# paulvoliva/XNODE-WAN-PDE-solver

Measured on AMD Instinct MI355X. Metric: WAN training-steps/sec (optimiser sub-steps, d=20 cube, N_r=4096 paths per GPU), higher is better.
Workload: dtype f64

## Files before the change

xnode_wan_pde_solver_amd/csrc/xw_ode_mfma4.h:

```cpp
#if XW_ODE_SECTION == 1
static_assert(XW_ODE_K <= 15, "row K of the 16-row K-tile is the ones row that collects the bias gradients");
static_assert(Dim<XW_ODE_H, XW_ODE_K>::HT <= 2 && Dim<XW_ODE_H, XW_ODE_K>::CT <= 3, "H <= 32");
template <int H, int K> struct FieldW {
  double Wy[Dim<H, K>::KB][Dim<H, K>::HB];
  double Wh[Dim<H, K>::KB][Dim<H, K>::KB];
  double Wo[Dim<H, K>::HB][Dim<H, K>::KB];
  d4 wt, bh;
  d4 bo[Dim<H, K>::HT];
};
template <int H, int K> struct FieldWT {
  double WyT[Dim<H, K>::HB][Dim<H, K>::KB];
  double WhT[Dim<H, K>::KB][Dim<H, K>::KB];
  double WoT[Dim<H, K>::KB][Dim<H, K>::HB];
};
template <int H, int K>
__device__ __forceinline__ void load_field(const double* __restrict__ th, const UOff& o, int d, FieldW<H, K>& w) {
  typedef Dim<H, K> D;
  const double* Wy = th + o.Win + d + 1;
#pragma unroll
  for (int rb = 0; rb < D::KB; ++rb) {
#pragma unroll
    for (int kb = 0; kb < D::HB; ++kb) w.Wy[rb][kb] = xw_fragA4(Wy, o.ldin, K, H, 4 * rb, 4 * kb);
#pragma unroll
    for (int kb = 0; kb < D::KB; ++kb) w.Wh[rb][kb] = xw_fragA4(th + o.Wh, K, K, K, 4 * rb, 4 * kb);
// ... 232 lines not shown
  const long col = (long)tile * 16 + 4 * k + b;
  const double* __restrict__ src_y = s.Yl + (long)row * N + (col < N - 1 ? col : N - 1);
  const double* __restrict__ src_a = s.A + (long)(AL::YI + (s.i > 0 ? s.i - 1 : 0) * H + 4 * cb) * 16 + lane;
  const xw_gptr src = row < H ? (xw_gptr)(first ? src_y : src_a) : (xw_gptr)&xw_duo_const[0][0];
  return __builtin_nontemporal_load(src);
}
__device__ __forceinline__ double duo_readA(const double* tile, int rb) {
  const int l = xw_lane();
  return tile[(4 * rb + (l & 3)) * XW_TSTRIDE + ((l >> 2) & 3) * 4 + (l >> 4)];
}
__device__ __forceinline__ double duo_fold(double x) {
  x += __shfl_xor(x, 4);
  x += __shfl_xor(x, 8);
  return x;
}
template <int H, int K, int M, int METHOD>
__device__ __forceinline__ void duo_outer(const BwdJobs& jobs, const double* __restrict__ tf, const double* __restrict__ th,
                                          int L, int d, const double* qbuf, int vb) {
  typedef Dim<H, K> D;
  typedef RK<METHOD> T;
  typedef DuoPlan<H, K, M> P;
  typedef Duo4<H, K, M> Q;
  typedef DuoSrc<H, K, M, METHOD> Src;
  constexpr int NH = M > 1 ? M - 1 : 1;
  xw_setprio(jobs.prio);
  const int job = find_job(jobs, vb);
  const double* __restrict__ Y = jobs.Y[job];
  const double* __restrict__ act = jobs.act[job];
  const int N = jobs.N[job];
  const int tile = vb - jobs.tile0[job];
  const int lane = xw_lane();
  const UOff o = u_offsets(d, H, K);
  double gWh[Q::KB][Q::KB1], gWo[Q::HB][Q::KB1], gWy[Q::KB][Q::HB1];
#pragma unroll
  for (int rb = 0; rb < Q::KB; ++rb) {
#pragma unroll
    for (int cb = 0; cb < Q::KB1; ++cb) gWh[rb][cb] = 0.0;
#pragma unroll
    for (int cb = 0; cb < Q::HB1; ++cb) gWy[rb][cb] = 0.0;
  }
#pragma unroll
  for (int rb = 0; rb < Q::HB; ++rb)
#pragma unroll
    for (int cb = 0; cb < Q::KB1; ++cb) gWo[rb][cb] = 0.0;
  double Ra[Q::KB1], Rr[NH][Q::KB1], Ry[Q::HB1];
  const int E = (L - 1) * T::S;
  double ti_cur = 0.0;
  if (E > 0) {
    const Src s0(Y, act, tf, 0, L, N, tile);
    ti_cur = s0.ti;
#pragma unroll
    for (int cb = 0; cb < Q::KB1; ++cb) Ra[cb] = duo_load_act<H, K, M, METHOD>(s0, M - 1, cb);
#pragma unroll
    for (int jj = M - 2; jj >= 0; --jj)
#pragma unroll
      for (int cb = 0; cb < Q::KB1; ++cb) Rr[jj][cb] = duo_load_act<H, K, M, METHOD>(s0, jj, cb);
#pragma unroll
    for (int cb = 0; cb < Q::HB1; ++cb) Ry[cb] = duo_load_y<H, K, M, METHOD>(s0, cb, N, tile);
  }
  const bool trow = (lane & 3) == (H & 3);
  for (int e = 0; e < E; ++e) {
    asm volatile("s_barrier" ::: "memory");
    const double* q = qbuf + (e & 1) * P::BUF;
    const Src sn(Y, act, tf, e + 1 < E ? e + 1 : e, L, N, tile);
    double Ao[Q::HB], Az[M][Q::KB];
#pragma unroll
    for (int rb = 0; rb < Q::HB; ++rb) Ao[rb] = duo_readA(q + P::off(rb >> 2), rb & 3);
#pragma unroll
    for (int tq = 0; tq < M; ++tq)
#pragma unroll
      for (int rb = 0; rb < Q::KB; ++rb) Az[tq][rb] = duo_readA(q + P::off(D::HT + tq), rb);
    __builtin_amdgcn_sched_barrier(0);
#pragma unroll
    for (int cb = 0; cb < Q::KB1; ++cb)
#pragma unroll
      for (int rb = 0; rb < Q::HB; ++rb) gWo[rb][cb] = XW_MFMA4(Ao[rb], Ra[cb], gWo[rb][cb]);
    __builtin_amdgcn_sched_barrier(0);
#pragma unroll
    for (int cb = 0; cb < Q::KB1; ++cb) Ra[cb] = duo_load_act<H, K, M, METHOD>(sn, M - 1, cb);
    __builtin_amdgcn_sched_barrier(0);
#pragma unroll
    for (int jj = M - 2; jj >= 0; --jj) {
#pragma unroll
      for (int cb = 0; cb < Q::KB1; ++cb)
#pragma unroll
        for (int rb = 0; rb < Q::KB; ++rb) gWh[rb][cb] = XW_MFMA4(Az[M - 2 - jj][rb], Rr[jj][cb], gWh[rb][cb]);
      __builtin_amdgcn_sched_barrier(0);
#pragma unroll
      for (int cb = 0; cb < Q::KB1; ++cb) Rr[jj][cb] = duo_load_act<H, K, M, METHOD>(sn, jj, cb);
      __builtin_amdgcn_sched_barrier(0);
    }
#pragma unroll
    for (int cb = 0; cb < Q::HB1; ++cb) {
      const double b = (cb == (H >> 2) && trow) ? ti_cur : Ry[cb];
#pragma unroll
      for (int rb = 0; rb < Q::KB; ++rb) gWy[rb][cb] = XW_MFMA4(Az[M - 1][rb], b, gWy[rb][cb]);
    }
    __builtin_amdgcn_sched_barrier(0);
#pragma unroll
    for (int cb = 0; cb < Q::HB1; ++cb) Ry[cb] = duo_load_y<H, K, M, METHOD>(sn, cb, N, tile);
    __builtin_amdgcn_sched_barrier(0);
    ti_cur = sn.ti;
  }
  double* slab = jobs.gslab[job] + (long)tile * o.total;
  const int i = lane >> 4, j = lane & 3;
  const bool owner = ((lane >> 2) & 3) == 0;
#pragma unroll
  for (int rb = 0; rb < Q::KB; ++rb)
#pragma unroll
    for (int cb = 0; cb < Q::KB1; ++cb) {
      const double x = duo_fold(gWh[rb][cb]);
      const int row = 4 * rb + i, col = 4 * cb + j;
      if (owner && row < K) {
        if (col < K) slab[o.Wh + row * K + col] = x;
        else if (col == K) slab[o.Whb + row] = x;
      }
    }
#pragma unroll
  for (int rb = 0; rb < Q::HB; ++rb)
#pragma unroll
    for (int cb = 0; cb < Q::KB1; ++cb) {
      const double x = duo_fold(gWo[rb][cb]);
      const int row = 4 * rb + i, col = 4 * cb + j;
      if (owner && row < H) {
        if (col < K) slab[o.Wo + row * K + col] = x;
        else if (col == K) slab[o.Wob + row] = x;
      }
    }
#pragma unroll
  for (int rb = 0; rb < Q::KB; ++rb)
#pragma unroll
    for (int cb = 0; cb < Q::HB1; ++cb) {
      const double x = duo_fold(gWy[rb][cb]);
      const int row = 4 * rb + i, col = 4 * cb + j;
      if (owner && row < K) {
        if (col < H) slab[o.Win + row * o.ldin + d + 1 + col] = x;
        else if (col == H) slab[o.Win + row * o.ldin + d] = x;
      }
    }
}
#elif XW_ODE_SECTION == 3
#include "xw_ode_n4.h"

template <int H, int K, int M>
bool launch_fwd_narrow(int sel, const FwdJobs& jobs, const double* t, const double* theta, int L, int d, dim3 grid, hipStream_t s, int& rc) {
  if (!jobs.narrow) return false;
  rc = XW_E_ARG;
// ... 6 lines not shown
    case 5: hipLaunchKernelGGL((n4::k_ode_fwd_n4<H, K, M, 1, 2>), grid, dim3(256), 0, s, jobs, t, theta, L, d); break;
    case 6: hipLaunchKernelGGL((n4::k_ode_fwd_n4<H, K, M, 2, 0>), grid, dim3(256), 0, s, jobs, t, theta, L, d); break;
    default: return true;
  }
  rc = xw_launch_status();
  return true;
}
template <int H, int K, int M, bool PARAMS>
int launch_bwd(int method, const BwdJobs& jobs, const double* t, const double* theta, int L, int d, bool adj, bool narrow,
               hipStream_t s) {
  const dim3 grid(jobs.tile0[jobs.n]), block(64);
  if (narrow) {
    if (adj || method > 1) return XW_E_ARG;
    for (int i = 0; i < jobs.n; ++i)
      if (jobs.act[i] == nullptr) return XW_E_ARG;
    if (method == 0) hipLaunchKernelGGL((n4::k_ode_bwd_n4<H, K, M, 0, PARAMS>), grid, dim3(256), 0, s, jobs, t, theta, L, d);
    else hipLaunchKernelGGL((n4::k_ode_bwd_n4<H, K, M, 1, PARAMS>), grid, dim3(256), 0, s, jobs, t, theta, L, d);
    return xw_launch_status();
  }
  bool act = true;
  for (int i = 0; i < jobs.n; ++i) act = act && jobs.act[i] != nullptr;
  if (adj || !act || method > 1)
    return XW_ODE_FN(xw_ode_bwd_recomp_w)(&jobs, t, theta, method, L, d, M, PARAMS ? 1 : 0, adj ? 1 : 0, (void*)s);
  static const int spread_on = [] { const char* e = getenv("XW_DUO_SPREAD"); return e ? atoi(e) : 1; }();
  static const int ncu = [] { int dev = 0, n = 0; if (hipGetDevice(&dev) != hipSuccess || hipDeviceGetAttribute(&n, hipDeviceAttributeMultiprocessorCount, dev) != hipSuccess) n = 0; return n; }();
  const int tiles = jobs.tile0[jobs.n];
  BwdJobs jd = jobs;
  jd.spread = (spread_on && ncu > 0 && tiles > ncu && tiles <= 2 * ncu) ? ncu : 0;
  const int rounds = jd.spread ? (tiles + ncu - 1) / ncu : 0;
  const dim3 duo_grid(jd.spread ? (2 * (rounds - 1)) * ncu + (tiles - (rounds - 1) * ncu) : tiles);
// ... 16 lines not shown
```

xnode_wan_pde_solver_amd/csrc/xw_ode_n4.h:

```cpp

namespace n4 {

template <int C> __device__ __forceinline__ int rot_i(int x) {
  if constexpr (C == 0) return x;
  else return __builtin_amdgcn_update_dpp(0, x, 0x120 + 4 * C, 0xf, 0xf, true);
}
template <int C> __device__ __forceinline__ double rot(double x) {
  if constexpr (C == 0) return x;
  else return __hiloint2double(rot_i<C>(__double2hiint(x)), rot_i<C>(__double2loint(x)));
}
struct R4 { double v[4]; };
__device__ __forceinline__ R4 rots(double x) { return R4{{x, rot<1>(x), rot<2>(x), rot<3>(x)}}; }

struct Geo {
  int lo, b, hi;
  int sb[4];
  int q;
};
__device__ __forceinline__ Geo geo() {
  Geo g;
  const int l = xw_lane();
  g.lo = l & 3; g.b = (l >> 2) & 3; g.hi = l >> 4;
  g.sb[0] = g.b; g.sb[1] = rot_i<1>(g.b); g.sb[2] = rot_i<2>(g.b); g.sb[3] = rot_i<3>(g.b);
  g.q = (int)(threadIdx.x >> 6);
// ... 103 lines not shown
  if (PARAMS) {
    R.aT = xw_ld_nt(S + (M - 1) * K * 16 + f.tK);
#pragma unroll
    for (int j = 0; j < M - 1; ++j) R.rT[j] = xw_ld_nt(S + j * K * 16 + f.tK);
    if (i == 0) {
#pragma unroll
      for (int y = 0; y < D::NY; ++y) R.yT[y] = xw_ld_g(Y + (long)l * H * N + yT[y]);
    } else {
#pragma unroll
      for (int y = 0; y < D::NY; ++y) R.yT[y] = xw_ld_nt(A + (long)(AL::YI + (i - 1) * H) * 16 + f.tY[y]);
    }
  }
  __builtin_amdgcn_sched_barrier(0);
}

template <int H, int K, int M, bool PARAMS>
__device__ __forceinline__ void vjp4(const WT4<H, K>& w, double eye, int blk, double t, const Stage4<H, K, M, PARAMS>& s,
                                     const double (&ob)[Dn<H, K>::NY], double (&yb)[Dn<H, K>::NY], double& xpb, Acc4<H, K>& G) {
  typedef Dn<H, K> D;
  __builtin_amdgcn_sched_barrier(0);
  const unsigned bits = s.word << blk;
  double ab = 0.0;
  {
    const R4 o0 = rots(ob[0]);
#pragma unroll
    for (int c = 0; c < 4; ++c) ab = XW_MFMA4(w.WoT0[c], o0.v[c], ab);
    if (D::NY == 2) {
      if (D::REP) ab = XW_MFMA4(w.WoT1[0], ob[D::NY - 1], ab);
      else {
        const R4 o1 = rots(ob[D::NY - 1]);
#pragma unroll
        for (int c = 0; c < 4; ++c) ab = XW_MFMA4(w.WoT1[c], o1.v[c], ab);
      }
    }
  }
  if (PARAMS) {
// ... 4 lines not shown
    G.bo[0] += ob[0];
    if (D::NY == 2) {
      const double q1 = XW_MFMA4(ob[D::NY - 1], eye, 0.0);
      if (D::REP) G.Wo1[0] = XW_MFMA4(q1, aT.v[0], G.Wo1[0]);
      else {
#pragma unroll
        for (int c = 0; c < 4; ++c) G.Wo1[c] = XW_MFMA4(q1, aT.v[c], G.Wo1[c]);
      }
      G.bo[D::NY - 1] += ob[D::NY - 1];
    }
  }
  double zb = ab * fma(-s.a, s.a, 1.0);
#pragma unroll
  for (int j = M - 2; j >= 0; --j) {
    const R4 zr = rots(zb);
    if (PARAMS) {
      const double qz = XW_MFMA4(zb, eye, 0.0);
      const R4 rT = rots(s.rT[j]);
#pragma unroll
      for (int c = 0; c < 4; ++c) G.Wh[c] = XW_MFMA4(qz, rT.v[c], G.Wh[c]);
      G.bh += zb;
    }
    double tt = 0.0;
#pragma unroll
    for (int c = 0; c < 4; ++c) tt = XW_MFMA4(w.WhT[c], zr.v[c], tt);
    zb = Stage4<H, K, M, PARAMS>::gate(bits, j, tt);
  }
  xpb += zb;
  const R4 zr = rots(zb);
  if (PARAMS) {
    const double qz = XW_MFMA4(zb, eye, 0.0);
    const R4 y0 = rots(s.yT[0]);
#pragma unroll
    for (int c = 0; c < 4; ++c) G.Wy0[c] = XW_MFMA4(qz, y0.v[c], G.Wy0[c]);
    if (D::NY == 2) {
      if (D::REP) G.Wy1[0] = XW_MFMA4(qz, s.yT[D::NY - 1], G.Wy1[0]);
      else {
        const R4 y1 = rots(s.yT[D::NY - 1]);
#pragma unroll
        for (int c = 0; c < 4; ++c) G.Wy1[c] = XW_MFMA4(qz, y1.v[c], G.Wy1[c]);
      }
    }
    G.wt = fma(t, zb, G.wt);
  }
#pragma unroll
  for (int y = 0; y < D::NY; ++y) yb[y] = 0.0;
#pragma unroll
  for (int c = 0; c < 4; ++c) {
    yb[0] = XW_MFMA4(w.WyT0[c], zr.v[c], yb[0]);
    if (D::NY == 2) yb[D::NY - 1] = XW_MFMA4(w.WyT1[c], zr.v[c], yb[D::NY - 1]);
  }
}

template <int H, int K> struct Plan4 {
  typedef Dn<H, K> D;
  static constexpr int NG = 12 + 2 * D::NC1;
  static constexpr int NTILE = 2 * D::NY + 2 + D::NY + 1;
  static constexpr int TILES = 0;
  static constexpr int HAND = TILES + XW_SWEEP_TILES * XW_TTILE;
  static constexpr int SCAL = HAND + NTILE * 256;
  static constexpr int GACC = SCAL + 32;
  static constexpr int TOTAL_P = GACC + 4 * NG * 64;
  static constexpr int TOTAL_X = SCAL + 32;
};

__device__ __forceinline__ void hand_over(double* tile, const Geo& g, double x, bool rep) {
  if (!rep) tile[64 * g.b + 16 * g.hi + 4 * g.q + g.lo] = x;
  else tile[64 * g.b + 16 * g.hi + 4 * g.q + g.lo] = g.b == 0 ? x : 0.0;
}
__device__ __forceinline__ d4 take_over(const double* tile) {
  const int l = xw_lane();
  d4 v;
#pragma unroll
  for (int r = 0; r < 4; ++r) v[r] = tile[64 * r + l];
  return v;
}
__device__ __forceinline__ void storeRowSumsStrided(double* dst, long stride, int rows, int r0, d4 q) {
  const int lane = xw_lane(), g = lane >> 4;
#pragma unroll
  for (int r = 0; r < 4; ++r) {
    const double s = xw_sum_over_n(q[r]);
    const int row = r0 + g + 4 * r;
    if ((lane & 15) == 0 && row < rows) dst[(long)row * stride] = s;
  }
}

template <int H, int K, int M, int METHOD, bool PARAMS>
__device__ __forceinline__ void sweep4(const BwdJobs& jobs, const double* __restrict__ tf, const double* __restrict__ th, int L, int d,
                                       double* lds, int vb) {
  typedef Dn<H, K> D;
  typedef Dim<H, K> DW;
  typedef RK<METHOD> T;
  typedef Plan4<H, K> P;
  static_assert(T::S <= 2, "the activation store is used by euler and midpoint");
  static_assert(D::NY == DW::HT, "registers of the hidden state = row tiles of the 16-path layout");
  xw_setprio(jobs.prio);
  const Geo g = geo();
  const int job = find_job(jobs, vb);
  const double* __restrict__ xT = jobs.xT[job];
  const double* __restrict__ start = jobs.start[job];
  const double* __restrict__ Y = jobs.Y[job];
  const double* __restrict__ act = jobs.act[job];
  const int N = jobs.N[job];
  const int tile = vb - jobs.tile0[job];
  const int base = tile * 16;
  const long ntile = (N + 15) >> 4;
  const int colC = base + 4 * g.q + g.lo, colT = base + 4 * g.q + g.hi;
  const bool valid = colC < N;
  const int nclC = valid ? colC : N - 1, nclT = colT < N ? colT : N - 1;
  const UOff o = u_offsets(d, H, K);
  WT4<H, K> w;
  load_WT4<H, K>(th, o, d, g, w);
  const Off4<H, K> f = offsets<H, K>(g);
  const double eye = g.lo == g.hi ? 1.0 : 0.0;
  int rowC[D::NY], rowT[D::NY];
  long yC[D::NY], yT[D::NY];
  double flw[D::NY];
#pragma unroll
  for (int y = 0; y < D::NY; ++y) {
    const int rc = y == 0 ? 4 * g.b + g.hi : (D::REP ? 16 + g.hi : 16 + 4 * g.b + g.hi);
    const int rt = y == 0 ? 4 * g.b + g.lo : (D::REP ? 16 + g.lo : 16 + 4 * g.b + g.lo);
    rowC[y] = rc;
    rowT[y] = rt;
    yC[y] = (long)(rc < H ? rc : H - 1) * N + nclC;
    yT[y] = (long)(rt < H ? rt : H - 1) * N + nclT;
    flw[y] = rc < H ? xw_ld_g(th + o.FLw + rc) : 0.0;
  }
  (void)rowT;

// ... 21 lines not shown
      if (PARAMS) accFL[y] = fma(ub, yl[y], accFL[y]);
    }
    if (PARAMS) accFLb += ub;
  };
  double kb[T::S][D::NY], psum[D::NY];
  auto begin_step = [&](int l) {
    const double dt = tf[l + 1] - tf[l];
#pragma unroll
    for (int i = 0; i < T::S; ++i)
#pragma unroll
      for (int y = 0; y < D::NY; ++y) {
        kb[i][y] = (dt * T::b(i)) * lam[y];
        if (i == 0) psum[y] = 0.0;
      }
  };
  auto reverse_stage = [&](int l, int i, const Stage4<H, K, M, PARAMS>& s) {
    const double t0 = tf[l], dt = tf[l + 1] - t0;
    double psi[D::NY];
    vjp4<H, K, M, PARAMS>(w, eye, g.b, t0 + T::c(i) * dt, s, kb[i], psi, xpb, G);
#pragma unroll
    for (int y = 0; y < D::NY; ++y) {
      psum[y] += psi[y];
#pragma unroll
      for (int j = 0; j < T::S; ++j)
        if (j < i && T::a(i, j) != 0.0) kb[j][y] = fma(dt * T::a(i, j), psi[y], kb[j][y]);
    }
  };
  auto end_step = [&](const double (&yl)[D::NY], double ub) {
#pragma unroll
    for (int y = 0; y < D::NY; ++y) lam[y] += psum[y];
    readout(yl, ub);
  };

  auto run = [&](auto weak_tag) {
    constexpr bool WEAK = decltype(weak_tag)::value;
    Stage4<H, K, M, PARAMS> sa, sb;
    const CotRaw raw_last = cot_issue<WEAK>(cot, L - 1);
    CotRaw raw = cot_issue<WEAK>(cot, L > 1 ? L - 2 : 0);
    if (L > 1) load_stage4<H, K, M, METHOD, PARAMS>(Y, act, L - 2, T::S - 1, N, ntile, tile, g, f, yT, sa);
    {
      double yl[D::NY];
      load_y(L - 1, yl);
      readout(yl, cot_value<WEAK>(cot, raw_last, L - 1, L));
    }
    for (int l = L - 2; l >= 0; --l) {
      const double ub = cot_value<WEAK>(cot, raw, l, L);
      double yl[D::NY];
      load_y(l, yl);
      if constexpr (T::S == 2) {
        load_stage4<H, K, M, METHOD, PARAMS>(Y, act, l, 0, N, ntile, tile, g, f, yT, sb);
        raw = cot_issue<WEAK>(cot, l > 0 ? l - 1 : 0);
        begin_step(l);
        reverse_stage(l, 1, sa);
        load_stage4<H, K, M, METHOD, PARAMS>(Y, act, l > 0 ? l - 1 : 0, 1, N, ntile, tile, g, f, yT, sa);
        reverse_stage(l, 0, sb);
      } else {
        sb = sa;
        raw = cot_issue<WEAK>(cot, l > 0 ? l - 1 : 0);
        load_stage4<H, K, M, METHOD, PARAMS>(Y, act, l > 0 ? l - 1 : 0, 0, N, ntile, tile, g, f, yT, sa);
        begin_step(l);
        reverse_stage(l, 0, sb);
      }
      end_step(yl, ub);
    }
  };
  if (cot.weak) run(std::true_type{});
  else run(std::false_type{});

  double* hand = lds + P::HAND;
#pragma unroll
  for (int y = 0; y < D::NY; ++y) {
    hand_over(hand + (0 * D::NY + y) * 256, g, lam[y], y == 1 && D::REP);
    if (PARAMS) {
      hand_over(hand + (1 * D::NY + y) * 256, g, accFL[y], y == 1 && D::REP);
      hand_over(hand + (2 * D::NY + 2 + y) * 256, g, G.bo[y], y == 1 && D::REP);
    }
  }
  hand_over(hand + (2 * D::NY) * 256, g, xpb, false);
  if (PARAMS) {
    hand_over(hand + (2 * D::NY + 1) * 256, g, G.bh, false);
    hand_over(hand + (3 * D::NY + 2) * 256, g, G.wt, false);
  }
  if (g.b == 0 && g.hi == 0) {
    lds[P::SCAL + 4 * g.q + g.lo] = ub0;
    lds[P::SCAL + 16 + 4 * g.q + g.lo] = accFLb;
  }
  if (PARAMS) {
    double* mine = lds + P::GACC + g.q * (P::NG * 64) + xw_lane();
    int r = 0;
#pragma unroll
    for (int c = 0; c < 4; ++c) mine[64 * (r++)] = G.Wh[c];
#pragma unroll
    for (int c = 0; c < 4; ++c) mine[64 * (r++)] = G.Wo0[c];
#pragma unroll
    for (int c = 0; c < 4; ++c) mine[64 * (r++)] = G.Wy0[c];
#pragma unroll
    for (int c = 0; c < D::NC1; ++c) mine[64 * (r++)] = G.Wo1[c];
#pragma unroll
    for (int c = 0; c < D::NC1; ++c) mine[64 * (r++)] = G.Wy1[c];
  }
  __syncthreads();
  double* slab = PARAMS ? jobs.gslab[job] + (long)tile * o.total : nullptr;
  if (PARAMS) {
    const double* all = lds + P::GACC + xw_lane();
    const int row = 4 * g.b + g.hi;
#pragma unroll
    for (int r = 0; r < P::NG; ++r) {
      if ((r & 3) != g.q) continue;
      const double x = (all[64 * r] + all[64 * (P::NG + r)]) + (all[64 * (2 * P::NG + r)] + all[64 * (3 * P::NG + r)]);
      const int kind = r < 12 ? r >> 2 : 3 + (r - 12) / (D::NC1 > 0 ? D::NC1 : 1);
      const int c = r < 12 ? r & 3 : (r - 12) % (D::NC1 > 0 ? D::NC1 : 1);
      const int col = 4 * g.sb[c] + g.lo;
      if (kind == 0) {
        if (row < K && col < K) slab[o.Wh + row * K + col] = x;
      } else if (kind == 1) {
        if (row < H && col < K) slab[o.Wo + row * K + col] = x;
      } else if (kind == 2) {
        if (row < K && col < H) slab[o.Win + row * o.ldin + d + 1 + col] = x;
// ... 8 lines not shown
  }
  if (g.q != 0) return;
  {
    const int lane = xw_lane(), n = lane & 15;
    const bool valid16 = base + n < N;
    const int ncl16 = valid16 ? base + n : N - 1;
    d4 lam16[DW::HT], fl16[DW::HT], flw16[DW::HT];
#pragma unroll
    for (int ht = 0; ht < DW::HT; ++ht) {
      lam16[ht] = take_over(hand + (0 * D::NY + ht) * 256);
      fl16[ht] = PARAMS ? take_over(hand + (1 * D::NY + ht) * 256) : xw_zero4();
      flw16[ht] = xw_vecD(th + o.FLw, H, 16 * ht);
    }
    const d4 xpb16 = take_over(hand + (2 * D::NY) * 256);
    const double ub016 = lds[P::SCAL + n], flb16 = lds[P::SCAL + 16 + n];
    if (PARAMS) {
      storeRowSums(slab + o.Whb, K, 0, take_over(hand + (2 * D::NY + 1) * 256));
#pragma unroll
      for (int ht = 0; ht < DW::HT; ++ht) storeRowSums(slab + o.Wob, H, 16 * ht, take_over(hand + (2 * D::NY + 2 + ht) * 256));
      storeRowSumsStrided(slab + o.Win + d, o.ldin, K, 0, take_over(hand + (3 * D::NY + 2) * 256));
    }
    sweep_tail<H, K, PARAMS, false>(th, o, d, N, base, valid16, ncl16, xT, start[ncl16], jobs.x_ones != 0, lam16, xpb16, ub016, fl16,
                                    flb16, flw16, jobs.gx[job], jobs.gs[job], slab, lds + P::TILES, []() {});
  }
}

template <int H, int K, int M, int METHOD, bool PARAMS>
__global__ void __launch_bounds__(256, 2) k_ode_bwd_n4(const BwdJobs jobs, const double* __restrict__ tf,
                                                       const double* __restrict__ th, int L, int d) {
  __shared__ double lds[PARAMS ? Plan4<H, K>::TOTAL_P : Plan4<H, K>::TOTAL_X];
  sweep4<H, K, M, METHOD, PARAMS>(jobs, tf, th, L, d, lds, (int)blockIdx.x);
}

template <int H, int K> struct W4 {
  double Wy0[4], Wy1[4], Wh[4], Wo0[4], Wo1[4];
  double wt, bh, bo[Dn<H, K>::NY];
};
template <int H, int K>
__device__ __forceinline__ void load_W4(const double* __restrict__ th, const UOff& o, int d, const Geo& g, W4<H, K>& w) {
  typedef Dn<H, K> D;
  const double* Wy = th + o.Win + d + 1;
  constexpr int H0 = H < 16 ? H : 16;
#pragma unroll
  for (int c = 0; c < 4; ++c) {
    w.Wy0[c] = frag<false>(Wy, o.ldin, K, H0, 0, 0, g, c);
    w.Wh[c] = frag<false>(th + o.Wh, K, K, K, 0, 0, g, c);
// ... 221 lines not shown
```

xnode_wan_pde_solver_amd/engine.py:

```python
import contextlib
import math
import os

import torch

from . import kernels as KN
from ._lib import XnwanError
from .options import EngineOptions
from .sampling import HIP_HOST_LOCK, _PIN_POOL, Hypercube, _paths


def ctypes_addr(fn):
    import ctypes
    return ctypes.cast(fn, ctypes.c_void_p).value

_KEPT_GRAPHS = []

_NOSTREAM = contextlib.nullcontext()

_SCRATCH_POOL = []


_DEVICE_STREAMS = {}

# ... 179 lines not shown
        self.use_runner = opt.use_runner
        if self.dopri5:
            self.use_graphs = self.use_streams = self.use_runner = self.keep_activations = False
        if self.tiled:
            self.use_runner = self.keep_activations = False
            self.narrow = '0'
        if self.testnet_tiled:
            self.use_runner = False
        self.narrow_set = str(opt.narrow_set)
        self.narrow_tiles = {'f': 192, 'x': 128, 'p': 64}
        if opt.narrow_tiles:
            self.narrow_tiles = dict(zip('fxp', (int(v_) for v_ in str(opt.narrow_tiles).split(':'))))
        self.narrow_tiles_alone = dict(zip('fxp', (int(v_) for v_ in str(opt.narrow_tiles_alone).split(':'))))
        for k_ in 'fxp':
            self.narrow_tiles_alone[k_] = max(self.narrow_tiles_alone[k_], self.narrow_tiles[k_])
        self.simds = 4 * cus
        self._phi_version = 0
        self.streams, self._cap = _device_streams(device)
        self.capture_exchange = (world is not None and getattr(world, 'capturable', False)
                                 and opt.capture_exchange)
        if self.capture_exchange:
            world.all_reduce(self.scal)

    def _tabulate_a(self, X1):
        d, dev, fa = self.d, self.dev, self.funcs['a']
        N = X1.shape[0]
        A = None
        try:
            ii = torch.arange(d, device=X1.device).view(d, 1, 1, 1)
            jj = torch.arange(d, device=X1.device).view(1, d, 1, 1)
# ... 633 lines not shown
            p = lambda t: 0 if t is None else t.data_ptr()
            xg.N, xg.Nb, xg.L, xg.Lb, xg.d = G.N, G.Nb, G.L, G.Lb, self.d
            xg.same_grid, xg.w_per_point, xg.amode = int(bool(G.same_grid)), int(G.w.dim() == 2), int(G.amode)
            xg.ns_u, xg.ns_b = G.ns_u, G.ns_b
            for k in ('xT', 'xvT', 'xbT', 't', 'tb', 'tpp', 'xvT_pts', 'start', 'start_b', 'h', 'href', 'f', 'g', 'w', 'wt', 'w0', 'ghT',
                      'gwx0T', 'A0', 'B0', 'u', 'Y', 'act', 'act_b', 'v', 'vt', 'gxv', 'gtv', 'gx', 'gs', 'vbar', 's3x', 'vact',
                      'xproj', 'slabA', 'slabB', 'slab_v', 'work_i', 'work_b', 'ub', 'Yb'):
                setattr(xg, k, G.ptr(k))
            nar = lambda jobs, **kw: self._narrow_ok(jobs, **kw)
            ji, jb = self._job(G, 'i'), (self._job(G, 'b') if G.Nb else None)
            joint = G.Nb and G.same_grid
            bits = [nar([ji] + ([jb] if joint else []), alone=False, forward=True),
                    bool(jb) and nar([jb], alone=False, forward=True),
                    nar([ji] + ([jb] if joint else []) + [ji], alone=False),
                    bool(jb) and nar([jb], alone=False),
                    bool(joint) and nar([ji, jb], alone=False),
                    nar([ji], alone=False, params=False),
                    nar([ji], alone=False, forward=True),
                    nar([ji], alone=False, params=False)]
            xg.narrow = sum(1 << i for i, b in enumerate(bits) if b)
        xg.sharded = int(bool(getattr(G, 'sharded', False)))
        xg.xproj_current = (2 if getattr(G, 'xproj_cur', False) else 1) if self._xproj_held(G) else 0
        xg.pair_i, xg.pair_b = int(bool(G.pair_i)), int(bool(G.pair_b))
        xg.Vol, xg.Nglob, xg.Nbglob, xg.s3_scale = float(G.Vol), float(G.Nglob), float(G.Nbglob), float(G.s3_scale)
        xg.init_off, xg.bdry_off, xg.ckappa = float(G.init_off), float(G.bdry_off), float(self.structure.c_kappa)
        xg.href = 0 if G.href is None else G.href.data_ptr()
        xg.c = xg.cp = 0
        return xg

    def _runner_ok(self, G):
        return (self.use_runner and self.structure.c_kappa is not None and G.c is None and not getattr(G, 'persistent', True))
# ... 4 lines not shown
    def _field_seen(self, G):
        touched = G.L > 1 or (getattr(G, 'has_bdry', G.Nb > 0) and G.Lb > 1)
        self._field_touched = touched or (self.accum_u is not None and self._field_touched)
        return self._field_touched

    def _narrow_ok(self, jobs, alone, forward=False, params=True):
        kind = 'f' if forward else ('p' if params else 'x')
        if self.narrow == '0' or kind not in self.narrow_set:
            return False
        if not forward and (self.adjoint or self.method > 1 or any(j.get('act') is None for j in jobs)):
            return False
        if self.narrow == '2':
            return True
        tiles = sum((j['xT'].shape[1] + 15) // 16 for j in jobs)
        return tiles <= (self.narrow_tiles_alone if alone else self.narrow_tiles)[kind]

    def _job(self, G, which, ubar=None, gslab=None, want_x=False):
        if which == 'i':
            j = dict(xT=G.xT, start=G.start, u=G.u, Y=G.Y, act=G.act, ubar=ubar, gslab=gslab)
            if want_x:
                j.update(gx=G.gx, gs=G.gs)
        else:
            j = dict(xT=G.xbT, start=G.start_b, u=G.ub, Y=G.Yb, act=G.act_b, ubar=ubar, gslab=gslab)
        return j

    def _res_init(self, G):
        return dict(u=G.u, ref=G.href if G.pair_i else G.h, coef=2.0 * self.alpha / G.Nglob, base=self.pollution, first_only=True)

    def _res_bdry(self, G):
        return dict(u=G.ub, ref=G.g, coef=2.0 * self.alpha / (G.Nbglob * G.Lb), base=0.0, first_only=False)
# ... 120 lines not shown
        if not lone:
            self._launch_test_net_here(G)
        with self._side(1, e0):
            fwd = [self._job(G, 'i'), self._job(G, 'b')]
            self._ode_fwd_multi(fwd, G.t, th, *M, zero16=self.scal, narrow=self._narrow_ok(fwd, alone=False, forward=True),
                             prio_drop=self.prio_drop['G'])
            self._reaction(G)
            sweep_x = [self._job(G, 'i', want_x=True)]
            self._ode_bwd_multi(sweep_x, G.t, th, *M, want_x=True, want_params=False,
                             narrow=self._narrow_ok(sweep_x, alone=False, params=False))
            e_x = self._mark()
        self._join(e_x)
        self._contract(G, self.adam_u, with_bdry=True)
        sweeps = [dict(self._job(G, 'i', None, G.slabA[:G.ns_u]), res=self._res_merged(G)),
                  dict(self._job(G, 'b', None, G.slabA[G.ns_u:]), res=self._res_bdry(G))]
        self._ode_bwd_multi(sweeps, G.t, th, *M, want_x=False, want_params=True, narrow=self._narrow_ok(sweeps, alone=False))
        G.sumA_ready = False

    def begin_substep(self, which, accumulate):
        name, P = ('accum_u', self.Pu) if which == 'u' else ('accum_v', self.Pv)
        if which == 'u':
            self._field_touched = False
        if not accumulate:
            setattr(self, name, None)
        elif getattr(self, name) is None:
            setattr(self, name, torch.zeros(P, dtype=F64, device=self.dev))
        else:
            getattr(self, name).zero_()

    def _gen_back(self, G):
        lr, st = self.config['u_rate'], self.adam_u
# ... 365 lines not shown
```

xnode_wan_pde_solver_amd/options.py:

```python
import dataclasses
import os
from typing import Optional


def _flag(name, default):
    v = os.environ.get(name)
    if v is None:
        return default
    return v != '0' if default else v == '1'


def _int(name, default):
    v = os.environ.get(name)
    return default if v in (None, '') else int(v)


@dataclasses.dataclass
class EngineOptions:
    use_streams: bool = True
    use_graphs: bool = True
    strict_graphs: bool = False
    reuse_test_net: bool = False
    keep_activations: bool = True
    v_blocks: int = 0
    v_blocks_disc: int = 0
    narrow: str = '1'
    narrow_set: str = 'fx'
    narrow_tiles: Optional[str] = None
    narrow_tiles_alone: str = '256:256:64'
    early_slab_sum: bool = True
    merged_sweep: bool = True
    compact_tiles: int = 320
    prio_drop_A: Optional[int] = None
    prio_drop_X: int = 0
    prio_drop_F: int = 0
    prio_drop_G: int = 0
    use_runner: bool = True
    capture_exchange: bool = True
    xproj_min_d: int = 45
    xproj_cached: bool = True
    xproj_cached_min_d: int = 20
    tiled_stepper: str = 'beyond'
    eval_chunk_paths: int = 65536
    hw_queues: int = 4
# ... 15 lines not shown

    @classmethod
    def from_env(cls):
        o = cls()
        o.use_streams = _flag('XW_STREAMS', o.use_streams)
        o.use_graphs = _flag('XW_GRAPHS', o.use_graphs)
        o.strict_graphs = _flag('XW_STRICT_GRAPHS', o.strict_graphs)
        o.reuse_test_net = _flag('XW_REUSE_V', o.reuse_test_net)
        o.keep_activations = _flag('XW_KEEP_ACT', o.keep_activations)
        o.v_blocks = _int('XW_V_BLOCKS', o.v_blocks)
        o.v_blocks_disc = _int('XW_V_BLOCKS_DISC', o.v_blocks_disc)
        o.narrow = os.environ.get('XW_NARROW', o.narrow)
        o.narrow_set = os.environ.get('XW_NARROW_SET', o.narrow_set)
        o.narrow_tiles = os.environ.get('XW_NARROW_TILES') or None
        o.narrow_tiles_alone = os.environ.get('XW_NARROW_TILES_ALONE') or o.narrow_tiles_alone
        o.early_slab_sum = _flag('XW_EARLY_SLAB_SUM', o.early_slab_sum)
        o.merged_sweep = _flag('XW_MERGED_SWEEP', o.merged_sweep)
        o.compact_tiles = _int('XW_COMPACT_TILES', o.compact_tiles)
        o.prio_drop_A = _int('XW_PRIO_DROP_A', None)
        o.prio_drop_X = _int('XW_PRIO_DROP_X', o.prio_drop_X)
        o.prio_drop_F = _int('XW_PRIO_DROP_F', o.prio_drop_F)
        o.prio_drop_G = _int('XW_PRIO_DROP_G', o.prio_drop_G)
        o.use_runner = _flag('XW_RUNNER', o.use_runner)
        o.capture_exchange = _flag('XW_CAPTURE_EXCHANGE', o.capture_exchange)
        o.xproj_min_d = _int('XW_XPROJ_MIN_D', o.xproj_min_d)
        o.xproj_cached = _flag('XW_XPROJ_CACHED', o.xproj_cached)
        o.xproj_cached_min_d = _int('XW_XPROJ_CACHED_MIN_D', o.xproj_cached_min_d)
        o.tiled_stepper = os.environ.get('XW_TILED_STEPPER') or o.tiled_stepper
        o.eval_chunk_paths = _int('XW_EVAL_CHUNK_PATHS', o.eval_chunk_paths)
        try:
# ... 24 lines not shown
```

Before: 2215.

## Split narrow backward sweep into chain waves plus partner outer-product waves

Adds a duo variant of the narrow backward ODE kernel. Four waves run the adjoint chain and post cotangents into double-buffered LDS, while one to four extra partner waves accumulate the weight-gradient outer products from those posts, each handling a column subset. The aim is to take the weight-gradient MFMA work off the serial chain's critical path. It also adds a separate tile threshold (narrow_tail, defaulting to the CU count) for routing the joint tail sweep to the narrow path. The cost is per-stage barriers and extra LDS traffic, and the tail routing rule now differs from the previous one.

```diff
diff --git a/xnode_wan_pde_solver_amd/csrc/xw_ode_mfma4.h b/xnode_wan_pde_solver_amd/csrc/xw_ode_mfma4.h
--- a/xnode_wan_pde_solver_amd/csrc/xw_ode_mfma4.h
+++ b/xnode_wan_pde_solver_amd/csrc/xw_ode_mfma4.h
@@ -270,7 +270,7 @@
   x += __shfl_xor(x, 8);
   return x;
 }
-template <int H, int K, int M, int METHOD>
+template <int H, int K, int M, int METHOD, bool TAILBAR = false, int NP = 1, int PART = 0>
 __device__ __forceinline__ void duo_outer(const BwdJobs& jobs, const double* __restrict__ tf, const double* __restrict__ th,
                                           int L, int d, const double* qbuf, int vb) {
   typedef Dim<H, K> D;
@@ -291,14 +291,14 @@
 #pragma unroll
   for (int rb = 0; rb < Q::KB; ++rb) {
 #pragma unroll
-    for (int cb = 0; cb < Q::KB1; ++cb) gWh[rb][cb] = 0.0;
-#pragma unroll
-    for (int cb = 0; cb < Q::HB1; ++cb) gWy[rb][cb] = 0.0;
+    for (int cb = PART; cb < Q::KB1; cb += NP) gWh[rb][cb] = 0.0;
+#pragma unroll
+    for (int cb = PART; cb < Q::HB1; cb += NP) gWy[rb][cb] = 0.0;
   }
 #pragma unroll
   for (int rb = 0; rb < Q::HB; ++rb)
 #pragma unroll
-    for (int cb = 0; cb < Q::KB1; ++cb) gWo[rb][cb] = 0.0;
+    for (int cb = PART; cb < Q::KB1; cb += NP) gWo[rb][cb] = 0.0;
   double Ra[Q::KB1], Rr[NH][Q::KB1], Ry[Q::HB1];
   const int E = (L - 1) * T::S;
   double ti_cur = 0.0;
@@ -306,13 +306,13 @@
     const Src s0(Y, act, tf, 0, L, N, tile);
     ti_cur = s0.ti;
 #pragma unroll
-    for (int cb = 0; cb < Q::KB1; ++cb) Ra[cb] = duo_load_act<H, K, M, METHOD>(s0, M - 1, cb);
+    for (int cb = PART; cb < Q::KB1; cb += NP) Ra[cb] = duo_load_act<H, K, M, METHOD>(s0, M - 1, cb);
 #pragma unroll
     for (int jj = M - 2; jj >= 0; --jj)
 #pragma unroll
-      for (int cb = 0; cb < Q::KB1; ++cb) Rr[jj][cb] = duo_load_act<H, K, M, METHOD>(s0, jj, cb);
-#pragma unroll
-    for (int cb = 0; cb < Q::HB1; ++cb) Ry[cb] = duo_load_y<H, K, M, METHOD>(s0, cb, N, tile);
+      for (int cb = PART; cb < Q::KB1; cb += NP) Rr[jj][cb] = duo_load_act<H, K, M, METHOD>(s0, jj, cb);
+#pragma unroll
+    for (int cb = PART; cb < Q::HB1; cb += NP) Ry[cb] = duo_load_y<H, K, M, METHOD>(s0, cb, N, tile);
   }
   const bool trow = (lane & 3) == (H & 3);
   for (int e = 0; e < E; ++e) {
@@ -328,43 +328,44 @@
       for (int rb = 0; rb < Q::KB; ++rb) Az[tq][rb] = duo_readA(q + P::off(D::HT + tq), rb);
     __builtin_amdgcn_sched_barrier(0);
 #pragma unroll
-    for (int cb = 0; cb < Q::KB1; ++cb)
+    for (int cb = PART; cb < Q::KB1; cb += NP)
 #pragma unroll
       for (int rb = 0; rb < Q::HB; ++rb) gWo[rb][cb] = XW_MFMA4(Ao[rb], Ra[cb], gWo[rb][cb]);
     __builtin_amdgcn_sched_barrier(0);
 #pragma unroll
-    for (int cb = 0; cb < Q::KB1; ++cb) Ra[cb] = duo_load_act<H, K, M, METHOD>(sn, M - 1, cb);
+    for (int cb = PART; cb < Q::KB1; cb += NP) Ra[cb] = duo_load_act<H, K, M, METHOD>(sn, M - 1, cb);
     __builtin_amdgcn_sched_barrier(0);
 #pragma unroll
     for (int jj = M - 2; jj >= 0; --jj) {
 #pragma unroll
-      for (int cb = 0; cb < Q::KB1; ++cb)
+      for (int cb = PART; cb < Q::KB1; cb += NP)
 #pragma unroll
         for (int rb = 0; rb < Q::KB; ++rb) gWh[rb][cb] = XW_MFMA4(Az[M - 2 - jj][rb], Rr[jj][cb], gWh[rb][cb]);
       __builtin_amdgcn_sched_barrier(0);
 #pragma unroll
-      for (int cb = 0; cb < Q::KB1; ++cb) Rr[jj][cb] = duo_load_act<H, K, M, METHOD>(sn, jj, cb);
+      for (int cb = PART; cb < Q::KB1; cb += NP) Rr[jj][cb] = duo_load_act<H, K, M, METHOD>(sn, jj, cb);
       __builtin_amdgcn_sched_barrier(0);
     }
 #pragma unroll
-    for (int cb = 0; cb < Q::HB1; ++cb) {
+    for (int cb = PART; cb < Q::HB1; cb += NP) {
       const double b = (cb == (H >> 2) && trow) ? ti_cur : Ry[cb];
 #pragma unroll
       for (int rb = 0; rb < Q::KB; ++rb) gWy[rb][cb] = XW_MFMA4(Az[M - 1][rb], b, gWy[rb][cb]);
     }
     __builtin_amdgcn_sched_barrier(0);
 #pragma unroll
-    for (int cb = 0; cb < Q::HB1; ++cb) Ry[cb] = duo_load_y<H, K, M, METHOD>(sn, cb, N, tile);
+    for (int cb = PART; cb < Q::HB1; cb += NP) Ry[cb] = duo_load_y<H, K, M, METHOD>(sn, cb, N, tile);
     __builtin_amdgcn_sched_barrier(0);
     ti_cur = sn.ti;
   }
+  if (TAILBAR) asm volatile("s_barrier" ::: "memory");
   double* slab = jobs.gslab[job] + (long)tile * o.total;
   const int i = lane >> 4, j = lane & 3;
   const bool owner = ((lane >> 2) & 3) == 0;
 #pragma unroll
   for (int rb = 0; rb < Q::KB; ++rb)
 #pragma unroll
-    for (int cb = 0; cb < Q::KB1; ++cb) {
+    for (int cb = PART; cb < Q::KB1; cb += NP) {
       const double x = duo_fold(gWh[rb][cb]);
       const int row = 4 * rb + i, col = 4 * cb + j;
       if (owner && row < K) {
@@ -375,7 +376,7 @@
 #pragma unroll
   for (int rb = 0; rb < Q::HB; ++rb)
 #pragma unroll
-    for (int cb = 0; cb < Q::KB1; ++cb) {
+    for (int cb = PART; cb < Q::KB1; cb += NP) {
       const double x = duo_fold(gWo[rb][cb]);
       const int row = 4 * rb + i, col = 4 * cb + j;
       if (owner && row < H) {
@@ -386,7 +387,7 @@
 #pragma unroll
   for (int rb = 0; rb < Q::KB; ++rb)
 #pragma unroll
-    for (int cb = 0; cb < Q::HB1; ++cb) {
+    for (int cb = PART; cb < Q::HB1; cb += NP) {
       const double x = duo_fold(gWy[rb][cb]);
       const int row = 4 * rb + i, col = 4 * cb + j;
       if (owner && row < K) {
@@ -423,6 +424,14 @@
     if (adj || method > 1) return XW_E_ARG;
     for (int i = 0; i < jobs.n; ++i)
       if (jobs.act[i] == nullptr) return XW_E_ARG;
+    static const int solo = [] { const char* e = getenv("XW_N4_SOLO"); return e ? atoi(e) : 0; }();
+    if constexpr (PARAMS) {
+      if (!solo) {
+        if (method == 0) hipLaunchKernelGGL((n4::k_ode_bwd_duo_n4<H, K, M, 0>), grid, dim3(n4::Duo4N<H, K, M>::THREADS), 0, s, jobs, t, theta, L, d);
+        else hipLaunchKernelGGL((n4::k_ode_bwd_duo_n4<H, K, M, 1>), grid, dim3(n4::Duo4N<H, K, M>::THREADS), 0, s, jobs, t, theta, L, d);
+        return xw_launch_status();
+      }
+    }
     if (method == 0) hipLaunchKernelGGL((n4::k_ode_bwd_n4<H, K, M, 0, PARAMS>), grid, dim3(256), 0, s, jobs, t, theta, L, d);
     else hipLaunchKernelGGL((n4::k_ode_bwd_n4<H, K, M, 1, PARAMS>), grid, dim3(256), 0, s, jobs, t, theta, L, d);
     return xw_launch_status();
diff --git a/xnode_wan_pde_solver_amd/csrc/xw_ode_n4.h b/xnode_wan_pde_solver_amd/csrc/xw_ode_n4.h
--- a/xnode_wan_pde_solver_amd/csrc/xw_ode_n4.h
+++ b/xnode_wan_pde_solver_amd/csrc/xw_ode_n4.h
@@ -141,12 +141,36 @@
   __builtin_amdgcn_sched_barrier(0);
 }
 
-template <int H, int K, int M, bool PARAMS>
+template <int H, int K, int M> struct Post4 { int t[DuoPlan<H, K, M>::NQ]; };
+template <int H, int K, int M> __device__ __forceinline__ Post4<H, K, M> post_offsets(const Geo& g) {
+  typedef DuoPlan<H, K, M> Q;
+  typedef Dn<H, K> D;
+  static_assert(16 * XW_TSTRIDE >= 256, "a spare slot per lane of the four chain waves");
+  Post4<H, K, M> p;
+  const int row = 4 * g.b + g.hi, col = 4 * g.lo + g.q;
+  const int spare = Q::BUF - 16 * XW_TSTRIDE + 64 * g.q + xw_lane();
+#pragma unroll
+  for (int t = 0; t < Q::NQ; ++t) {
+    const int rows = t < Q::HT - 1 ? 16 : (t == Q::HT - 1 ? Q::HLAST : Q::KROWS);
+    const bool rep = D::REP && t == 1;
+    const bool live = rep ? g.b == 0 : row < rows;
+    p.t[t] = live ? Q::off(t) + (rep ? g.hi : row) * XW_TSTRIDE + col : spare;
+  }
+  return p;
+}
+
+template <int H, int K, int M, bool PARAMS, bool POST = false>
 __device__ __forceinline__ void vjp4(const WT4<H, K>& w, double eye, int blk, double t, const Stage4<H, K, M, PARAMS>& s,
-                                     const double (&ob)[Dn<H, K>::NY], double (&yb)[Dn<H, K>::NY], double& xpb, Acc4<H, K>& G) {
-  typedef Dn<H, K> D;
+                                     const double (&ob)[Dn<H, K>::NY], double (&yb)[Dn<H, K>::NY], double& xpb, Acc4<H, K>& G,
+                                     double* qb = nullptr, const Post4<H, K, M>* pt = nullptr) {
+  typedef Dn<H, K> D;
+  static_assert(!(PARAMS && POST), "a wave either contracts its own outer products or posts for the partner");
   __builtin_amdgcn_sched_barrier(0);
   const unsigned bits = s.word << blk;
+  if (POST) {
+#pragma unroll
+    for (int y = 0; y < D::NY; ++y) qb[pt->t[y]] = ob[y];
+  }
   double ab = 0.0;
   {
     const R4 o0 = rots(ob[0]);
@@ -181,6 +205,7 @@
 #pragma unroll
   for (int j = M - 2; j >= 0; --j) {
     const R4 zr = rots(zb);
+    if (POST) qb[pt->t[D::NY + (M - 2 - j)]] = zb;
     if (PARAMS) {
       const double qz = XW_MFMA4(zb, eye, 0.0);
       const R4 rT = rots(s.rT[j]);
@@ -195,6 +220,7 @@
   }
   xpb += zb;
   const R4 zr = rots(zb);
+  if (POST) qb[pt->t[D::NY + M - 1]] = zb;
   if (PARAMS) {
     const double qz = XW_MFMA4(zb, eye, 0.0);
     const R4 y0 = rots(s.yT[0]);
@@ -219,12 +245,12 @@
   }
 }
 
-template <int H, int K> struct Plan4 {
+template <int H, int K, bool DUO = false> struct Plan4 {
   typedef Dn<H, K> D;
   static constexpr int NG = 12 + 2 * D::NC1;
-  static constexpr int NTILE = 2 * D::NY + 2 + D::NY + 1;
+  static constexpr int NTILE = DUO ? 2 * D::NY + 1 : 2 * D::NY + 2 + D::NY + 1;
   static constexpr int TILES = 0;
-  static constexpr int HAND = TILES + XW_SWEEP_TILES * XW_TTILE;
+  static constexpr int HAND = DUO ? 0 : TILES + XW_SWEEP_TILES * XW_TTILE;
   static constexpr int SCAL = HAND + NTILE * 256;
   static constexpr int GACC = SCAL + 32;
   static constexpr int TOTAL_P = GACC + 4 * NG * 64;
@@ -252,13 +278,17 @@
   }
 }
 
-template <int H, int K, int M, int METHOD, bool PARAMS>
+template <int H, int K, int M, int METHOD, bool PARAMS, bool DUO = false>
 __device__ __forceinline__ void sweep4(const BwdJobs& jobs, const double* __restrict__ tf, const double* __restrict__ th, int L, int d,
-                                       double* lds, int vb) {
+                                       double* lds, int vb, double* qbuf = nullptr) {
+  static_assert(!DUO || PARAMS, "the duo sweep is a sweep with weight gradients");
   typedef Dn<H, K> D;
   typedef Dim<H, K> DW;
   typedef RK<METHOD> T;
-  typedef Plan4<H, K> P;
+  typedef Plan4<H, K, DUO> P;
+  constexpr bool OUTER = PARAMS && !DUO;
+  int qflip = 0;
+  Post4<H, K, M> pt;
   static_assert(T::S <= 2, "the activation store is used by euler and midpoint");
   static_assert(D::NY == DW::HT, "registers of the hidden state = row tiles of the 16-path layout");
   xw_setprio(jobs.prio);
@@ -280,6 +310,7 @@
   load_WT4<H, K>(th, o, d, g, w);
   const Off4<H, K> f = offsets<H, K>(g);
   const double eye = g.lo == g.hi ? 1.0 : 0.0;
+  if constexpr (DUO) pt = post_offsets<H, K, M>(g);
   int rowC[D::NY], rowT[D::NY];
   long yC[D::NY], yT[D::NY];
   double flw[D::NY];
@@ -331,10 +362,16 @@
         if (i == 0) psum[y] = 0.0;
       }
   };
-  auto reverse_stage = [&](int l, int i, const Stage4<H, K, M, PARAMS>& s) {
+  auto reverse_stage = [&](int l, int i, const Stage4<H, K, M, OUTER>& s) {
     const double t0 = tf[l], dt = tf[l + 1] - t0;
     double psi[D::NY];
-    vjp4<H, K, M, PARAMS>(w, eye, g.b, t0 + T::c(i) * dt, s, kb[i], psi, xpb, G);
+    if constexpr (DUO) {
+      vjp4<H, K, M, false, true>(w, eye, g.b, t0 + T::c(i) * dt, s, kb[i], psi, xpb, G, qbuf + qflip * DuoPlan<H, K, M>::BUF, &pt);
+      asm volatile("s_waitcnt lgkmcnt(0)\n\ts_barrier" ::: "memory");
+      qflip ^= 1;
+    } else {
+      vjp4<H, K, M, PARAMS>(w, eye, g.b, t0 + T::c(i) * dt, s, kb[i], psi, xpb, G);
+    }
 #pragma unroll
     for (int y = 0; y < D::NY; ++y) {
       psum[y] += psi[y];
@@ -351,10 +388,10 @@
 
   auto run = [&](auto weak_tag) {
     constexpr bool WEAK = decltype(weak_tag)::value;
-    Stage4<H, K, M, PARAMS> sa, sb;
+    Stage4<H, K, M, OUTER> sa, sb;
     const CotRaw raw_last = cot_issue<WEAK>(cot, L - 1);
     CotRaw raw = cot_issue<WEAK>(cot, L > 1 ? L - 2 : 0);
-    if (L > 1) load_stage4<H, K, M, METHOD, PARAMS>(Y, act, L - 2, T::S - 1, N, ntile, tile, g, f, yT, sa);
+    if (L > 1) load_stage4<H, K, M, METHOD, OUTER>(Y, act, L - 2, T::S - 1, N, ntile, tile, g, f, yT, sa);
     {
       double yl[D::NY];
       load_y(L - 1, yl);
@@ -365,16 +402,16 @@
       double yl[D::NY];
       load_y(l, yl);
       if constexpr (T::S == 2) {
-        load_stage4<H, K, M, METHOD, PARAMS>(Y, act, l, 0, N, ntile, tile, g, f, yT, sb);
+        load_stage4<H, K, M, METHOD, OUTER>(Y, act, l, 0, N, ntile, tile, g, f, yT, sb);
         raw = cot_issue<WEAK>(cot, l > 0 ? l - 1 : 0);
         begin_step(l);
         reverse_stage(l, 1, sa);
-        load_stage4<H, K, M, METHOD, PARAMS>(Y, act, l > 0 ? l - 1 : 0, 1, N, ntile, tile, g, f, yT, sa);
+        load_stage4<H, K, M, METHOD, OUTER>(Y, act, l > 0 ? l - 1 : 0, 1, N, ntile, tile, g, f, yT, sa);
         reverse_stage(l, 0, sb);
       } else {
         sb = sa;
         raw = cot_issue<WEAK>(cot, l > 0 ? l - 1 : 0);
-        load_stage4<H, K, M, METHOD, PARAMS>(Y, act, l > 0 ? l - 1 : 0, 0, N, ntile, tile, g, f, yT, sa);
+        load_stage4<H, K, M, METHOD, OUTER>(Y, act, l > 0 ? l - 1 : 0, 0, N, ntile, tile, g, f, yT, sa);
         begin_step(l);
         reverse_stage(l, 0, sb);
       }
@@ -388,13 +425,11 @@
 #pragma unroll
   for (int y = 0; y < D::NY; ++y) {
     hand_over(hand + (0 * D::NY + y) * 256, g, lam[y], y == 1 && D::REP);
-    if (PARAMS) {
-      hand_over(hand + (1 * D::NY + y) * 256, g, accFL[y], y == 1 && D::REP);
-      hand_over(hand + (2 * D::NY + 2 + y) * 256, g, G.bo[y], y == 1 && D::REP);
-    }
+    if (PARAMS) hand_over(hand + (1 * D::NY + y) * 256, g, accFL[y], y == 1 && D::REP);
+    if (OUTER) hand_over(hand + (2 * D::NY + 2 + y) * 256, g, G.bo[y], y == 1 && D::REP);
   }
   hand_over(hand + (2 * D::NY) * 256, g, xpb, false);
-  if (PARAMS) {
+  if (OUTER) {
     hand_over(hand + (2 * D::NY + 1) * 256, g, G.bh, false);
     hand_over(hand + (3 * D::NY + 2) * 256, g, G.wt, false);
   }
@@ -402,7 +437,7 @@
     lds[P::SCAL + 4 * g.q + g.lo] = ub0;
     lds[P::SCAL + 16 + 4 * g.q + g.lo] = accFLb;
   }
-  if (PARAMS) {
+  if (OUTER) {
     double* mine = lds + P::GACC + g.q * (P::NG * 64) + xw_lane();
     int r = 0;
 #pragma unroll
@@ -416,9 +451,10 @@
 #pragma unroll
     for (int c = 0; c < D::NC1; ++c) mine[64 * (r++)] = G.Wy1[c];
   }
-  __syncthreads();
+  if (DUO) asm volatile("s_waitcnt lgkmcnt(0)\n\ts_barrier" ::: "memory");
+  else __syncthreads();
   double* slab = PARAMS ? jobs.gslab[job] + (long)tile * o.total : nullptr;
-  if (PARAMS) {
+  if (OUTER) {
     const double* all = lds + P::GACC + xw_lane();
     const int row = 4 * g.b + g.hi;
 #pragma unroll
@@ -457,14 +493,15 @@
     }
     const d4 xpb16 = take_over(hand + (2 * D::NY) * 256);
     const double ub016 = lds[P::SCAL + n], flb16 = lds[P::SCAL + 16 + n];
-    if (PARAMS) {
+    if (OUTER) {
       storeRowSums(slab + o.Whb, K, 0, take_over(hand + (2 * D::NY + 1) * 256));
 #pragma unroll
       for (int ht = 0; ht < DW::HT; ++ht) storeRowSums(slab + o.Wob, H, 16 * ht, take_over(hand + (2 * D::NY + 2 + ht) * 256));
       storeRowSumsStrided(slab + o.Win + d, o.ldin, K, 0, take_over(hand + (3 * D::NY + 2) * 256));
     }
     sweep_tail<H, K, PARAMS, false>(th, o, d, N, base, valid16, ncl16, xT, start[ncl16], jobs.x_ones != 0, lam16, xpb16, ub016, fl16,
-                                    flb16, flw16, jobs.gx[job], jobs.gs[job], slab, lds + P::TILES, []() {});
+                                    flb16, flw16, jobs.gx[job], jobs.gs[job], slab,
+                                    DUO ? qbuf + qflip * DuoPlan<H, K, M>::BUF : lds + P::TILES, []() {});
   }
 }
 
@@ -473,6 +510,25 @@
                                                        const double* __restrict__ th, int L, int d) {
   __shared__ double lds[PARAMS ? Plan4<H, K>::TOTAL_P : Plan4<H, K>::TOTAL_X];
   sweep4<H, K, M, METHOD, PARAMS>(jobs, tf, th, L, d, lds, (int)blockIdx.x);
+}
+
+template <int H, int K, int M> struct Duo4N {
+  static constexpr int NP = Duo4<H, K, M>::KB1;
+  static_assert(NP >= 1 && NP <= 4, "partner waves");
+  static constexpr int THREADS = 64 * (4 + NP);
+};
+template <int H, int K, int M, int METHOD>
+__global__ void __launch_bounds__((Duo4N<H, K, M>::THREADS)) k_ode_bwd_duo_n4(const BwdJobs jobs, const double* __restrict__ tf,
+                                                                            const double* __restrict__ th, int L, int d) {
+  typedef DuoPlan<H, K, M> Q;
+  constexpr int NP = Duo4N<H, K, M>::NP;
+  __shared__ double lds[2 * Q::BUF + Plan4<H, K, true>::TOTAL_X];
+  const int wv = (int)(threadIdx.x >> 6), vb = (int)blockIdx.x;
+  if (wv < 4) sweep4<H, K, M, METHOD, true, true>(jobs, tf, th, L, d, lds + 2 * Q::BUF, vb, lds);
+  else if (wv == 4) duo_outer<H, K, M, METHOD, true, NP, 0>(jobs, tf, th, L, d, lds, vb);
+  else if (NP > 1 && wv == 5) duo_outer<H, K, M, METHOD, true, NP, (NP > 1 ? 1 : 0)>(jobs, tf, th, L, d, lds, vb);
+  else if (NP > 2 && wv == 6) duo_outer<H, K, M, METHOD, true, NP, (NP > 2 ? 2 : 0)>(jobs, tf, th, L, d, lds, vb);
+  else if (NP > 3 && wv == 7) duo_outer<H, K, M, METHOD, true, NP, (NP > 3 ? 3 : 0)>(jobs, tf, th, L, d, lds, vb);
 }
 
 template <int H, int K> struct W4 {
diff --git a/xnode_wan_pde_solver_amd/engine.py b/xnode_wan_pde_solver_amd/engine.py
--- a/xnode_wan_pde_solver_amd/engine.py
+++ b/xnode_wan_pde_solver_amd/engine.py
@@ -217,6 +217,7 @@
         self.narrow_tiles_alone = dict(zip('fxp', (int(v_) for v_ in str(opt.narrow_tiles_alone).split(':'))))
         for k_ in 'fxp':
             self.narrow_tiles_alone[k_] = max(self.narrow_tiles_alone[k_], self.narrow_tiles[k_])
+        self.narrow_tail = int(opt.narrow_tail) if int(opt.narrow_tail) >= 0 else int(cus)
         self.simds = 4 * cus
         self._phi_version = 0
         self.streams, self._cap = _device_streams(device)
@@ -880,7 +881,7 @@
                     bool(jb) and nar([jb], alone=False, forward=True),
                     nar([ji] + ([jb] if joint else []) + [ji], alone=False),
                     bool(jb) and nar([jb], alone=False),
-                    bool(joint) and nar([ji, jb], alone=False),
+                    bool(joint) and self._narrow_tail_ok([ji, jb]),
                     nar([ji], alone=False, params=False),
                     nar([ji], alone=False, forward=True),
                     nar([ji], alone=False, params=False)]
@@ -915,6 +916,13 @@
             return True
         tiles = sum((j['xT'].shape[1] + 15) // 16 for j in jobs)
         return tiles <= (self.narrow_tiles_alone if alone else self.narrow_tiles)[kind]
+
+    def _narrow_tail_ok(self, jobs):
+        if self.narrow == '0' or self.narrow_tail <= 0:
+            return False
+        if self.adjoint or self.method > 1 or any(j.get('act') is None for j in jobs):
+            return False
+        return sum((j['xT'].shape[1] + 15) // 16 for j in jobs) <= self.narrow_tail
 
     def _job(self, G, which, ubar=None, gslab=None, want_x=False):
         if which == 'i':
@@ -1065,7 +1073,7 @@
         self._contract(G, self.adam_u, with_bdry=True)
         sweeps = [dict(self._job(G, 'i', None, G.slabA[:G.ns_u]), res=self._res_merged(G)),
                   dict(self._job(G, 'b', None, G.slabA[G.ns_u:]), res=self._res_bdry(G))]
-        self._ode_bwd_multi(sweeps, G.t, th, *M, want_x=False, want_params=True, narrow=self._narrow_ok(sweeps, alone=False))
+        self._ode_bwd_multi(sweeps, G.t, th, *M, want_x=False, want_params=True, narrow=self._narrow_tail_ok(sweeps))
         G.sumA_ready = False
 
     def begin_substep(self, which, accumulate):
diff --git a/xnode_wan_pde_solver_amd/options.py b/xnode_wan_pde_solver_amd/options.py
--- a/xnode_wan_pde_solver_amd/options.py
+++ b/xnode_wan_pde_solver_amd/options.py
@@ -28,6 +28,7 @@
     narrow_set: str = 'fx'
     narrow_tiles: Optional[str] = None
     narrow_tiles_alone: str = '256:256:64'
+    narrow_tail: int = -1
     early_slab_sum: bool = True
     merged_sweep: bool = True
     compact_tiles: int = 320
@@ -73,6 +74,7 @@
         o.narrow_set = os.environ.get('XW_NARROW_SET', o.narrow_set)
         o.narrow_tiles = os.environ.get('XW_NARROW_TILES') or None
         o.narrow_tiles_alone = os.environ.get('XW_NARROW_TILES_ALONE') or o.narrow_tiles_alone
+        o.narrow_tail = _int('XW_NARROW_TAIL', o.narrow_tail)
         o.early_slab_sum = _flag('XW_EARLY_SLAB_SUM', o.early_slab_sum)
         o.merged_sweep = _flag('XW_MERGED_SWEEP', o.merged_sweep)
         o.compact_tiles = _int('XW_COMPACT_TILES', o.compact_tiles)
```

Measured after the change: 2205. About the same (-0.5%).
